# selkies-project/selkies

Measured on NVIDIA H100. Metric: 4K frames/sec encoded, higher is better.
Workload: dtype u8

## Files before the change

### selkies_b200/csrc/b2v_api.cu

```cuda
#include <condition_variable>
#include <cstdarg>
#include <cstdio>
#include <cstring>
#include <deque>
#include <mutex>
#include <thread>
#include <vector>

#include <sys/prctl.h>
#include <time.h>

#include "../../include/b2video.h"
#include "b2v_internal.h"
#include "h264_encoder.h"
#include "jpeg.h"

using namespace b2v;

static thread_local char g_err[512] = "";
static int fail(int code, const char* fmt, ...) {
  va_list ap; va_start(ap, fmt); vsnprintf(g_err, sizeof g_err, fmt, ap); va_end(ap);
  return code;
}
#define CK(call)                                                                              \
  do { cudaError_t e_ = (call);                                                               \
       if (e_ != cudaSuccess) return fail(B2V_ECUDA, "%s -> %s (%s:%d)", #call, cudaGetErrorString(e_), __FILE__, __LINE__); \
  } while (0)

namespace {

constexpr int kMaxSlots = 16;
constexpr int kOutHead = 64;
constexpr size_t kFirstChunk = 256 << 10;

struct Job {
  int out_idx; int in_slot; int frame_id; int is_key; int64_t capture_ns; int64_t pts; int hdr_w, hdr_h;
  bool timing;
};

inline int64_t now_ns() {
  timespec ts; clock_gettime(CLOCK_MONOTONIC, &ts);
  return (int64_t)ts.tv_sec * 1000000000LL + ts.tv_nsec;
}

constexpr int64_t kSpinNs = 30000, kSleepNs = 25000, kGiveUpNs = 30LL * 1000000000LL;
inline cudaError_t wait_event_polling(cudaEvent_t ev, bool* slept) {
  const int64_t t0 = now_ns();
  for (;;) {
    const cudaError_t e = cudaEventQuery(ev);
    if (e != cudaErrorNotReady) return e;
    const int64_t waited = now_ns() - t0;
    if (waited < kSpinNs) {
      for (int i = 0; i < 16; i++) __builtin_ia32_pause();
    } else if (waited > kGiveUpNs) {
      return cudaErrorLaunchTimeout;
    } else {
      *slept = true;
      timespec ts{0, (long)kSleepNs};
      nanosleep(&ts, nullptr);
    }
  }
}

enum : uint8_t { SLOT_FREE = 0, SLOT_ACQUIRED = 1, SLOT_IN_FLIGHT = 2 };

struct Session {
  b2v_settings cfg{};
  int device = 0;
  int src_w = 0, src_h = 0, dst_w = 0, dst_h = 0, coded_w = 0, coded_h = 0;
  bool encode = true, timing = false, timing_csc_only = false;
  cudaStream_t st_copy = nullptr, st_enc = nullptr, st_out = nullptr, st_pack = nullptr;

  int n_slots = 4;
  uint8_t* host_slot[kMaxSlots] = {};
  uint8_t* dev_slot[kMaxSlots] = {};
  cudaEvent_t ev_h2d[kMaxSlots] = {};
  uint8_t slot_state[kMaxSlots] = {};
  size_t frame_bytes = 0;
  std::vector<uint8_t*> resident;
  Tap *d_tx = nullptr, *d_ty = nullptr;
  uint8_t* d_cur = nullptr;
  Encoder* enc = nullptr;
  JpegEncoder* jenc = nullptr;
  bool jpeg = false;
  uint8_t* d_au[kMaxSlots] = {};
  uint8_t* h_out[kMaxSlots] = {};
  cudaEvent_t ev_enc[kMaxSlots] = {}, ev_out[kMaxSlots] = {};
  bool out_free[kMaxSlots] = {};
  AuLayout lay{};
  int out_next = 0;
  int ring_next = 0;
  cudaEvent_t ev_timer[2] = {};
  unsigned long long* d_csc_ts = nullptr;

  uint32_t frame_id = 0;
  int64_t frames_since_idr = 0;
  bool want_idr = true;
  double fps = 60.0;
  int bitrate_kbps = 8000;
  int qp_fixed = 26;

  cudaEvent_t ev_t[kMaxSlots][6] = {};

  b2v_cb cb = nullptr; void* user = nullptr;
  std::mutex mu;
  std::mutex submit_mu;
  std::condition_variable cv_slot, cv_job, cv_done;
  std::deque<Job> jobs;
  int64_t submitted = 0, delivered = 0;
  bool stopping = false;
  bool resizing = false;
  bool failed = false; char fail_msg[256] = "";
  std::thread out_thread;
  b2v_stats stats{};
};

int round16(int v) { return (v + 15) & ~15; }

bool size_ok(int w, int h) { return w >= 16 && h >= 16 && w <= 7680 && h <= 4320 && !(w & 1) && !(h & 1); }

int alloc_geometry(Session* s) {
  s->coded_w = s->encode ? round16(s->dst_w) : s->dst_w;
  s->coded_h = s->encode ? round16(s->dst_h) : s->dst_h;
  s->frame_bytes = (size_t)s->src_w * s->src_h * 4;
  for (int i = 0; i < s->n_slots; i++) {
    CK(cudaHostAlloc((void**)&s->host_slot[i], s->frame_bytes, cudaHostAllocDefault));
    CK(cudaMalloc((void**)&s->dev_slot[i], s->frame_bytes));
    s->slot_state[i] = SLOT_FREE;
  }
  CK(cudaMalloc((void**)&s->d_cur, (size_t)s->coded_w * s->coded_h * 3 / 2));
  if (s->dst_w != s->src_w || s->dst_h != s->src_h) {
    std::vector<Tap> tx(s->dst_w), ty(s->dst_h);
    make_taps_host(tx.data(), s->dst_w, s->src_w);
    make_taps_host(ty.data(), s->dst_h, s->src_h);
    CK(cudaMalloc((void**)&s->d_tx, sizeof(Tap) * s->dst_w));
    CK(cudaMalloc((void**)&s->d_ty, sizeof(Tap) * s->dst_h));
    CK(cudaMemcpy(s->d_tx, tx.data(), sizeof(Tap) * s->dst_w, cudaMemcpyHostToDevice));
    CK(cudaMemcpy(s->d_ty, ty.data(), sizeof(Tap) * s->dst_h, cudaMemcpyHostToDevice));
  }
  if (s->encode && s->jpeg) {
    JpegConfig jc{};
    jc.width = s->dst_w; jc.height = s->dst_h; jc.coded_w = s->coded_w; jc.coded_h = s->coded_h;
    jc.stripe_rows = s->cfg.stripe_rows > 0 ? s->cfg.stripe_rows : (s->coded_h / 16 + 7) / 8;
    jc.quality = s->cfg.crf > 0 ? s->cfg.crf : 60; jc.paint_quality = s->cfg.paintover_crf > 0 ? s->cfg.paintover_crf : 90;
    jc.paint_trigger = s->cfg.paintover_trigger_frames > 0 ? s->cfg.paintover_trigger_frames : 0;
    int rc = jpeg_create(&jc, &s->jenc);
    if (rc) return fail(rc, "jpeg_create failed: %s", jpeg_last_error());
    s->lay = jpeg_layout(s->jenc);
  } else if (s->encode) {
    EncoderConfig ec{};
    ec.width = s->dst_w; ec.height = s->dst_h; ec.coded_w = s->coded_w; ec.coded_h = s->coded_h;
    ec.slice_rows = s->cfg.slice_rows;
    ec.stripe_rows = s->cfg.stripe_rows > 0 ? s->cfg.stripe_rows : 0;
    ec.idr_slice_mbs = s->cfg.idr_slice_mbs;
    int rc = encoder_create(&ec, &s->enc);
    if (rc) return fail(rc, "encoder_create failed: %s", encoder_last_error());
    s->lay = encoder_layout(s->enc);
  }
  for (int i = 0; i < s->n_slots; i++) {
    if (s->encode) {
      CK(cudaMalloc((void**)&s->d_au[i], s->lay.cap));
      CK(cudaHostAlloc((void**)&s->h_out[i], s->lay.cap + kOutHead, cudaHostAllocDefault));
    }
    s->out_free[i] = true;
  }
  return 0;
}

void free_geometry(Session* s) {
  for (int i = 0; i < kMaxSlots; i++) {
    if (s->host_slot[i]) cudaFreeHost(s->host_slot[i]);
    if (s->dev_slot[i]) cudaFree(s->dev_slot[i]);
    if (s->d_au[i]) cudaFree(s->d_au[i]);
    if (s->h_out[i]) cudaFreeHost(s->h_out[i]);
    s->host_slot[i] = s->dev_slot[i] = s->d_au[i] = s->h_out[i] = nullptr;
  }
  for (auto p : s->resident) if (p) cudaFree(p);
  s->resident.clear();
  if (s->d_cur) cudaFree(s->d_cur);
  if (s->d_tx) cudaFree(s->d_tx);
  if (s->d_ty) cudaFree(s->d_ty);
  s->d_cur = nullptr; s->d_tx = nullptr; s->d_ty = nullptr;
  if (s->enc) { encoder_destroy(s->enc); s->enc = nullptr; }
  if (s->jenc) { jpeg_destroy(s->jenc); s->jenc = nullptr; }
}

CscParams csc_params(Session* s, const uint8_t* d_bgra, int stride, uint8_t* d_nv12) {
  CscParams p{};
  p.src = d_bgra; p.src_w = s->src_w; p.src_h = s->src_h; p.src_stride = stride;
  p.dst_w = s->dst_w; p.dst_h = s->dst_h; p.coded_w = s->coded_w; p.coded_h = s->coded_h;
  p.out_y = d_nv12; p.out_uv = d_nv12 + (size_t)s->coded_w * s->coded_h;
  p.tx = s->d_tx; p.ty = s->d_ty;
  p.matrix = s->jpeg ? 1 : 0;
  return p;
}

int wait_au(Session* s, const Job& j, int64_t* ns_event, bool* slept) {
  const int64_t tw = now_ns();
  const cudaError_t se = wait_event_polling(s->encode ? s->ev_out[j.out_idx] : s->ev_enc[j.out_idx], slept);
  *ns_event = now_ns() - tw;
  if (!s->encode) return 0;
  uint8_t* base = s->h_out[j.out_idx];
  const AuHeader* ah = (const AuHeader*)base;
  const int size = ah->size;
  const size_t doff = (size_t)s->lay.data_off;
  if (se != cudaSuccess || size < 0 || (size_t)size + doff > s->lay.cap || ah->overflow) {
    std::lock_guard<std::mutex> lk(s->mu);
    if (!s->failed) snprintf(s->fail_msg, sizeof s->fail_msg, "encode pipeline failed on frame %d: %s (size %d, overflow %d)", j.frame_id,
                             se != cudaSuccess ? cudaGetErrorString(se) : "invalid access unit", size, ah->overflow);
    s->failed = true;
    return 0;
  }
  if ((size_t)size + doff > kFirstChunk && size > 0) {
    size_t have = kFirstChunk;
    cudaMemcpyAsync(base + have, s->d_au[j.out_idx] + have, doff + (size_t)size - have, cudaMemcpyDeviceToHost, s->st_out);
    cudaStreamSynchronize(s->st_out);
    std::lock_guard<std::mutex> lk(s->mu);
    s->stats.d2h_bytes += (int64_t)(doff + size - have);
  }
  return size;
}

void add_timing(Session* s, const Job& j, bool have_au) {
  cudaEvent_t* ev = s->ev_t[j.out_idx];
  float ms[6] = {0, 0, 0, 0, 0, 0};
  cudaEventElapsedTime(&ms[0], ev[0], ev[1]);
  const bool stages = s->encode && !s->timing_csc_only;
  if (stages) {
    for (int k = 1; k < 5; k++) cudaEventElapsedTime(&ms[k], ev[k], ev[k + 1]);
    cudaEventElapsedTime(&ms[5], ev[0], ev[5]);
  } else ms[5] = ms[0];
  std::lock_guard<std::mutex> lk(s->mu);
  s->stats.ms_csc += ms[0]; s->stats.n_csc++;
  if (have_au) {
    const AuHeader* ah = (const AuHeader*)s->h_out[j.out_idx];
    if (ah->csc_t1 > ah->csc_t0 && ah->csc_t0 != 0) { s->stats.ms_csc_device += (double)(ah->csc_t1 - ah->csc_t0) * 1e-6; s->stats.n_csc_device++; }
  }
  if (stages) {
    if (j.is_key) { s->stats.ms_intra += ms[1]; s->stats.n_intra++; }
    else { s->stats.ms_inter += ms[1]; s->stats.n_inter++; }
    s->stats.ms_cavlc += ms[2]; s->stats.n_cavlc++;
    s->stats.ms_slice += ms[3]; s->stats.n_slice++;
    s->stats.ms_pack += ms[4]; s->stats.n_pack++;
  }
  s->stats.ms_total_gpu += ms[5];
}

void put_pixelflux_header(uint8_t* h, const Job& j, int y0, int bh) {
  h[0] = 0x04; h[1] = j.is_key ? 1 : 0;
  h[2] = (uint8_t)(j.frame_id >> 8); h[3] = (uint8_t)j.frame_id;
  h[4] = (uint8_t)(y0 >> 8); h[5] = (uint8_t)y0;
  h[6] = (uint8_t)(j.hdr_w >> 8); h[7] = (uint8_t)j.hdr_w;
  h[8] = (uint8_t)(bh >> 8); h[9] = (uint8_t)bh;
}

int64_t deliver(Session* s, const Job& j, int size, std::vector<BandEntry>& tab, int64_t* ns_cb) {
  uint8_t* base = s->h_out[j.out_idx];
  uint8_t* au = base + s->lay.data_off;
  const int qp = ((const AuHeader*)base)->qp;
  int rows = j.hdr_h;
  if (s->lay.n_bands == 0) {
    tab.assign(1, BandEntry{0, size, 1, 0});
  } else {
    tab.resize(s->lay.n_bands);
    memcpy(tab.data(), base + sizeof(AuHeader), sizeof(BandEntry) * s->lay.n_bands);
    rows = s->lay.band_rows * 16;
  }
  const bool hdr = s->cfg.header_mode == B2V_HDR_PIXELFLUX;
  int64_t bytes = 0;
  for (int b = 0; b < (int)tab.size(); b++) {
    const BandEntry& be = tab[b];
    if (!be.coded || be.size <= 0 || (long long)be.off + be.size > size) continue;
    const int y0 = b * rows, bh = (y0 + rows <= j.hdr_h) ? rows : j.hdr_h - y0;
    b2v_frame f{};
    f.data = au + be.off; f.size = be.size;
    if (hdr && s->jpeg) {
      uint8_t* h = au + be.off - 4;
      h[0] = (uint8_t)(j.frame_id >> 8); h[1] = (uint8_t)j.frame_id; h[2] = (uint8_t)(y0 >> 8); h[3] = (uint8_t)y0;
      f.data = h; f.size += 4;
    } else if (hdr) {
      put_pixelflux_header(au + be.off - 10, j, y0, bh);
      f.data = au + be.off - 10; f.size += 10;
    }
    f.frame_id = j.frame_id; f.is_key = j.is_key; f.qp = qp; f.pts90k = j.pts; f.capture_ns = j.capture_ns;
    f.y_start = y0; f.height = bh;
    bytes += f.size;
    if (s->cb) { const int64_t tc = now_ns(); s->cb(&f, s->user); *ns_cb += now_ns() - tc; }
  }
  return bytes;
}

void output_loop(Session* s) {
  cudaSetDevice(s->device);
  prctl(PR_SET_TIMERSLACK, 1000UL, 0, 0, 0);
  std::vector<BandEntry> tab;
  for (;;) {
    Job j;
    {
      std::unique_lock<std::mutex> lk(s->mu);
      if (s->jobs.empty() && !s->stopping) {
        const int64_t t0 = now_ns();
        s->cv_job.wait(lk, [&] { return s->stopping || !s->jobs.empty(); });
        s->stats.ns_wait_job += now_ns() - t0;
      }
      if (s->jobs.empty()) { if (s->stopping) return; continue; }
      j = s->jobs.front(); s->jobs.pop_front();
    }
    int64_t ns_event = 0, ns_cb = 0, bytes = 0; bool slept = false;
    const int size = wait_au(s, j, &ns_event, &slept);
    if (j.timing) add_timing(s, j, size > 0);
    if (size > 0) bytes = deliver(s, j, size, tab, &ns_cb);
    {
      std::lock_guard<std::mutex> lk(s->mu);
      if (j.in_slot >= 0) s->slot_state[j.in_slot] = SLOT_FREE;
      s->out_free[j.out_idx] = true;
      s->delivered++;
      s->stats.frames_delivered++;
      s->stats.bytes_out += bytes;
      if (j.is_key) s->stats.key_frames++;
      s->stats.ns_wait_event += ns_event; s->stats.ns_callback += ns_cb;
      if (ns_event > s->stats.ns_wait_event_max) s->stats.ns_wait_event_max = ns_event;
      if (slept) s->stats.n_event_sleeps++;
    }
    s->cv_slot.notify_all();
    s->cv_done.notify_all();
  }
}

int submit_failed(Session* s, int out_idx, int in_slot, cudaError_t e, const char* what) {
  {
    std::lock_guard<std::mutex> lk(s->mu);
    if (!s->failed) snprintf(s->fail_msg, sizeof s->fail_msg, "%s -> %s", what, cudaGetErrorString(e));
    s->failed = true;
    if (out_idx >= 0) { s->out_free[out_idx] = true; s->submitted--; s->stats.frames_submitted--; }
    if (in_slot >= 0) s->slot_state[in_slot] = SLOT_FREE;
  }
  s->cv_slot.notify_all(); s->cv_done.notify_all();
  return fail(B2V_ECUDA, "%s", s->fail_msg);
}
#define CKS(call)                                                                              \
  do { cudaError_t e_ = (call); if (e_ != cudaSuccess) return submit_failed(s, out_idx, in_slot, e_, #call); } while (0)

int submit_common(Session* s, const uint8_t* d_bgra, int stride, int in_slot, int64_t capture_ns) {
  int out_idx = 0;
  Job j{};
  EncodeFrameParams fp{};
  const int64_t t_enter = now_ns();
  int64_t t_slot = 0;
  {
    std::unique_lock<std::mutex> lk(s->mu);
    out_idx = s->out_next;
    s->cv_slot.wait(lk, [&] { return s->out_free[out_idx] || s->stopping || s->failed; });
    if (s->failed || s->stopping) {
      if (in_slot >= 0) s->slot_state[in_slot] = SLOT_FREE;
      lk.unlock(); s->cv_slot.notify_all();
      return s->failed ? fail(B2V_ECUDA, "%s", s->fail_msg) : fail(B2V_ESTATE, "session is stopping");
    }
    t_slot = now_ns() - t_enter;
    s->stats.ns_wait_out_slot += t_slot;
    s->out_free[out_idx] = false;
    s->out_next = (s->out_next + 1) % s->n_slots;
    bool idr = s->want_idr || (s->cfg.gop > 0 && s->frames_since_idr >= s->cfg.gop);
    s->want_idr = false;
    s->frames_since_idr = idr ? 1 : s->frames_since_idr + 1;
    j.out_idx = out_idx; j.in_slot = in_slot; j.frame_id = (int)(s->frame_id & 0xffff); j.is_key = idr;
    j.capture_ns = capture_ns;
    int ifps = (int)s->fps; if (ifps < 1) ifps = 1;
    j.pts = (int64_t)j.frame_id * (90000 / ifps);
    j.hdr_w = s->dst_w; j.hdr_h = s->dst_h;
    j.timing = s->timing && (!s->timing_csc_only || (s->frame_id & 3) == 0);
    s->frame_id++;
    fp.idr = idr;
    fp.rc_mode = s->cfg.rc_mode;
    fp.qp_fixed = s->qp_fixed;
    fp.paint_trigger = s->cfg.paintover_trigger_frames > 0 ? s->cfg.paintover_trigger_frames : 0;
    fp.paint_qp = s->cfg.paintover_crf;
    fp.paint_burst = s->cfg.paintover_burst_frames > 0 ? s->cfg.paintover_burst_frames : 1;
    fp.target_bits = (int64_t)((double)s->bitrate_kbps * 1000.0 / (s->fps > 0 ? s->fps : 60.0));
    s->submitted++;
    s->stats.frames_submitted++;
  }
  CscParams cp = csc_params(s, d_bgra, stride, s->d_cur);
  cudaEvent_t* ev = j.timing ? s->ev_t[out_idx] : nullptr;
  if (ev && s->d_csc_ts && s->encode) {
    cp.ts = s->d_csc_ts + 2 * out_idx;
    cudaMemsetAsync(cp.ts, 0xFF, sizeof(unsigned long long), s->st_enc);
    cudaMemsetAsync(cp.ts + 1, 0, sizeof(unsigned long long), s->st_enc);
  }
  if (ev) cudaEventRecord(ev[0], s->st_enc);
  int nl = launch_csc(cp, s->st_enc);
  if (ev) cudaEventRecord(ev[1], s->st_enc);
  cudaStream_t st_done = s->st_enc;
  if (s->encode && s->jpeg) {
    nl += jpeg_encode(s->jenc, s->d_cur, s->d_au[out_idx], j.is_key, s->st_enc);
  } else if (s->encode) {
    fp.cur = s->d_cur; fp.au = s->d_au[out_idx]; fp.ev = s->timing_csc_only ? nullptr : ev; fp.csc_ts = cp.ts;
    fp.st_pack = fp.ev ? nullptr : s->st_pack;
    nl += encoder_encode(s->enc, &fp, s->st_enc);
    if (fp.st_pack) st_done = fp.st_pack;
  }
  CKS(cudaEventRecord(s->ev_enc[out_idx], st_done));
  if (s->encode) {
    CKS(cudaStreamWaitEvent(s->st_out, s->ev_enc[out_idx], 0));
    const size_t first = s->lay.cap < kFirstChunk ? s->lay.cap : kFirstChunk;
    CKS(cudaMemcpyAsync(s->h_out[out_idx], s->d_au[out_idx], first, cudaMemcpyDeviceToHost, s->st_out));
    CKS(cudaEventRecord(s->ev_out[out_idx], s->st_out));
    std::lock_guard<std::mutex> lk(s->mu);
    s->stats.d2h_bytes += (int64_t)first;
  }
  CKS(cudaGetLastError());
  {
    std::lock_guard<std::mutex> lk(s->mu);
    s->stats.kernel_launches += nl;
    s->stats.ns_submit += now_ns() - t_enter - t_slot;
    s->jobs.push_back(j);
  }
  s->cv_job.notify_one();
  return 0;
}

void release_session(Session* s) {
  cudaSetDevice(s->device);
  cudaDeviceSynchronize();
  free_geometry(s);
  for (int i = 0; i < kMaxSlots; i++) {
    if (s->ev_h2d[i]) cudaEventDestroy(s->ev_h2d[i]);
    if (s->ev_enc[i]) cudaEventDestroy(s->ev_enc[i]);
    if (s->ev_out[i]) cudaEventDestroy(s->ev_out[i]);
    for (cudaEvent_t e : s->ev_t[i]) if (e) cudaEventDestroy(e);
  }
  if (s->ev_timer[0]) cudaEventDestroy(s->ev_timer[0]);
  if (s->ev_timer[1]) cudaEventDestroy(s->ev_timer[1]);
  if (s->d_csc_ts) cudaFree(s->d_csc_ts);
  if (s->st_copy) cudaStreamDestroy(s->st_copy);
  if (s->st_enc) cudaStreamDestroy(s->st_enc);
  if (s->st_out) cudaStreamDestroy(s->st_out);
  if (s->st_pack) cudaStreamDestroy(s->st_pack);
  delete s;
}

int bench_csc(Session* s, int32_t n_resident, int32_t iters, float* ms_per_launch, bool burst) {
  if (!s || n_resident <= 0 || n_resident > (int)s->resident.size() || iters <= 0 || !ms_per_launch) return fail(B2V_EINVAL, "bad argument");
  int rc = b2v_flush(s);
  if (rc) return rc;
  std::lock_guard<std::mutex> sub(s->submit_mu);
  CK(cudaSetDevice(s->device));
  std::vector<uint8_t*> outs(n_resident, nullptr);
  size_t ob = (size_t)s->coded_w * s->coded_h * 3 / 2;
  for (auto& o : outs) CK(cudaMalloc((void**)&o, ob));
  for (int i = 0; i < n_resident; i++) launch_csc(csc_params(s, s->resident[i], s->src_w * 4, outs[i]), s->st_enc);
  CK(cudaStreamSynchronize(s->st_enc));
  const int pairs = burst ? 1 : iters;
  std::vector<cudaEvent_t> e0(pairs), e1(pairs);
  for (int i = 0; i < pairs; i++) { cudaEventCreate(&e0[i]); cudaEventCreate(&e1[i]); }
  if (burst) cudaEventRecord(e0[0], s->st_enc);
  for (int i = 0; i < iters; i++) {
    int k = i % n_resident;
    if (!burst) cudaEventRecord(e0[i], s->st_enc);
    launch_csc(csc_params(s, s->resident[k], s->src_w * 4, outs[k]), s->st_enc);
    if (!burst) cudaEventRecord(e1[i], s->st_enc);
  }
  if (burst) cudaEventRecord(e1[0], s->st_enc);
  CK(cudaStreamSynchronize(s->st_enc));
  double total = 0;
  for (int i = 0; i < pairs; i++) { float ms = 0; cudaEventElapsedTime(&ms, e0[i], e1[i]); total += ms; cudaEventDestroy(e0[i]); cudaEventDestroy(e1[i]); }
  for (auto o : outs) cudaFree(o);
  CK(cudaGetLastError());
  *ms_per_launch = (float)(total / iters);
  return 0;
}

}

extern "C" {

int b2v_abi_version(void) { return B2V_ABI_VERSION; }
const char* b2v_last_error(void) { return g_err; }

int b2v_device_count(void) {
  int n = 0;
  if (cudaGetDeviceCount(&n) != cudaSuccess) return 0;
  return n;
}

int b2v_create(const b2v_settings* cfg, b2v_cb cb, void* user, void** out) {
  if (!cfg || !out) return fail(B2V_EINVAL, "null argument");
  int sw = cfg->src_w, sh = cfg->src_h;
  int dw = cfg->dst_w > 0 ? cfg->dst_w : sw, dh = cfg->dst_h > 0 ? cfg->dst_h : sh;
  if (!size_ok(sw, sh)) return fail(B2V_EINVAL, "source size %dx%d unsupported (even, 16..7680 x 16..4320)", sw, sh);
  if (!size_ok(dw, dh)) return fail(B2V_EINVAL, "encoded size %dx%d unsupported", dw, dh);
  if (cfg->idr_slice_mbs < 0) return fail(B2V_EINVAL, "idr_slice_mbs %d out of range (0 = default, n > 0 macroblocks per slice)", cfg->idr_slice_mbs);
  int ndev = 0;
  CK(cudaGetDeviceCount(&ndev));
  if (cfg->device < 0 || cfg->device >= ndev) return fail(B2V_EINVAL, "device %d out of range (%d devices)", cfg->device, ndev);
  CK(cudaSetDevice(cfg->device));
  Session* s = new Session();
  s->cfg = *cfg; s->device = cfg->device;
  s->src_w = sw; s->src_h = sh; s->dst_w = dw; s->dst_h = dh;
  s->encode = !(cfg->flags & B2V_FLAG_NO_ENCODE);
  s->jpeg = (cfg->flags & B2V_FLAG_JPEG) != 0;
  s->timing = (cfg->flags & (B2V_FLAG_TIMING | B2V_FLAG_TIMING_CSC)) != 0;
  s->timing_csc_only = s->timing && !(cfg->flags & B2V_FLAG_TIMING);
  s->n_slots = cfg->ring_slots > 0 ? cfg->ring_slots : 4;
  if (s->n_slots < 2) s->n_slots = 2;
  if (s->n_slots > kMaxSlots) s->n_slots = kMaxSlots;
  s->fps = cfg->fps > 0 ? cfg->fps : 60.0;
  s->bitrate_kbps = cfg->bitrate_kbps > 0 ? cfg->bitrate_kbps : 8000;
  s->qp_fixed = cfg->crf >= 0 ? cfg->crf : 26;
  if (s->qp_fixed > 51) s->qp_fixed = 51;
  s->cb = cb; s->user = user;
  cudaStreamCreateWithFlags(&s->st_copy, cudaStreamNonBlocking);
  cudaStreamCreateWithFlags(&s->st_enc, cudaStreamNonBlocking);
  cudaStreamCreateWithFlags(&s->st_out, cudaStreamNonBlocking);
  cudaStreamCreateWithFlags(&s->st_pack, cudaStreamNonBlocking);
  for (int i = 0; i < kMaxSlots; i++) {
    cudaEventCreateWithFlags(&s->ev_h2d[i], cudaEventDisableTiming);
    cudaEventCreateWithFlags(&s->ev_enc[i], cudaEventDisableTiming);
    cudaEventCreateWithFlags(&s->ev_out[i], cudaEventDisableTiming);
  }
  for (auto& evs : s->ev_t) for (cudaEvent_t& e : evs) cudaEventCreate(&e);
  cudaEventCreate(&s->ev_timer[0]); cudaEventCreate(&s->ev_timer[1]);
  if (s->timing && (cfg->flags & B2V_FLAG_DEVICE_TIMER)) cudaMalloc((void**)&s->d_csc_ts, sizeof(unsigned long long) * 2 * kMaxSlots);
  int rc = alloc_geometry(s);
  if (rc) { release_session(s); return rc; }
  s->out_thread = std::thread(output_loop, s);
  *out = s;
  return 0;
}

void b2v_destroy(void* h) {
  if (!h) return;
  Session* s = (Session*)h;
  b2v_flush(h);
  {
    std::lock_guard<std::mutex> lk(s->mu);
    s->stopping = true;
  }
  s->cv_job.notify_all(); s->cv_slot.notify_all();
  if (s->out_thread.joinable()) s->out_thread.join();
  release_session(s);
}

void* b2v_ring_acquire(void* h, int32_t* slot) {
  Session* s = (Session*)h;
  if (!s || !slot) { fail(B2V_EINVAL, "null argument"); return nullptr; }
  std::unique_lock<std::mutex> lk(s->mu);
  if ((s->resizing || s->slot_state[s->ring_next] != SLOT_FREE) && !s->stopping && !s->failed) {
    const int64_t t0 = now_ns();
    s->cv_slot.wait(lk, [&] { return s->stopping || s->failed || (!s->resizing && s->slot_state[s->ring_next] == SLOT_FREE); });
    s->stats.ns_wait_ring += now_ns() - t0;
  }
  if (s->failed) { fail(B2V_ECUDA, "%s", s->fail_msg); return nullptr; }
  if (s->stopping) { fail(B2V_ESTATE, "session is stopping"); return nullptr; }
  const int found = s->ring_next;
  s->ring_next = (found + 1) % s->n_slots;
  s->slot_state[found] = SLOT_ACQUIRED;
  *slot = found;
  return s->host_slot[found];
}

int b2v_ring_release(void* h, int32_t slot) {
  Session* s = (Session*)h;
  if (!s || slot < 0 || slot >= s->n_slots) return fail(B2V_EINVAL, "bad slot");
  {
    std::lock_guard<std::mutex> lk(s->mu);
    if (s->slot_state[slot] != SLOT_ACQUIRED || (slot + 1) % s->n_slots != s->ring_next) return fail(B2V_ESTATE, "slot %d is not the most recently acquired one", slot);
    s->slot_state[slot] = SLOT_FREE;
    s->ring_next = slot;
  }
  s->cv_slot.notify_all();
  return 0;
}

int b2v_ring_submit(void* h, int32_t slot, int32_t stride, int64_t capture_ns) {
  Session* s = (Session*)h;
  if (!s || slot < 0 || slot >= s->n_slots) return fail(B2V_EINVAL, "bad slot");
  if (stride <= 0) stride = s->src_w * 4;
  if (stride < s->src_w * 4 || (size_t)stride * s->src_h > s->frame_bytes) return fail(B2V_EINVAL, "stride %d does not fit the slot", stride);
  std::lock_guard<std::mutex> sub(s->submit_mu);
  {
    std::lock_guard<std::mutex> lk(s->mu);
    if (s->slot_state[slot] != SLOT_ACQUIRED) return fail(B2V_ESTATE, "slot %d was not acquired (double submit?)", slot);
    s->slot_state[slot] = SLOT_IN_FLIGHT;
  }
  const int64_t t0 = now_ns();
  const int out_idx = -1, in_slot = slot;
  CKS(cudaSetDevice(s->device));
  CKS(cudaMemcpyAsync(s->dev_slot[slot], s->host_slot[slot], (size_t)stride * s->src_h, cudaMemcpyHostToDevice, s->st_copy));
  CKS(cudaEventRecord(s->ev_h2d[slot], s->st_copy));
  CKS(cudaStreamWaitEvent(s->st_enc, s->ev_h2d[slot], 0));
  {
    std::lock_guard<std::mutex> lk(s->mu);
    s->stats.h2d_bytes += (int64_t)stride * s->src_h;
    s->stats.ns_submit += now_ns() - t0;
  }
  return submit_common(s, s->dev_slot[slot], stride, slot, capture_ns);
}

int b2v_resident_upload(void* h, int32_t index, const void* bgra, int32_t stride) {
  Session* s = (Session*)h;
  if (!s || index < 0 || index >= 1024 || !bgra) return fail(B2V_EINVAL, "bad argument");
  if (stride <= 0) stride = s->src_w * 4;
  std::lock_guard<std::mutex> sub(s->submit_mu);
  CK(cudaSetDevice(s->device));
  if ((int)s->resident.size() <= index) s->resident.resize(index + 1, nullptr);
  if (!s->resident[index]) CK(cudaMalloc((void**)&s->resident[index], s->frame_bytes));
  CK(cudaMemcpy2D(s->resident[index], (size_t)s->src_w * 4, bgra, stride, (size_t)s->src_w * 4, s->src_h, cudaMemcpyHostToDevice));
  return 0;
}

int b2v_submit_resident(void* h, int32_t index, int64_t capture_ns) {
  Session* s = (Session*)h;
  if (!s || index < 0 || index >= (int)s->resident.size() || !s->resident[index]) return fail(B2V_EINVAL, "resident frame %d not uploaded", index);
  std::lock_guard<std::mutex> sub(s->submit_mu);
  CK(cudaSetDevice(s->device));
  return submit_common(s, s->resident[index], s->src_w * 4, -1, capture_ns);
}

int b2v_flush(void* h) {
  Session* s = (Session*)h;
  if (!s) return fail(B2V_EINVAL, "null handle");
  std::unique_lock<std::mutex> lk(s->mu);
  s->cv_done.wait(lk, [&] { return s->delivered >= s->submitted; });
  if (s->failed) return fail(B2V_ECUDA, "%s", s->fail_msg);
  return 0;
}

int b2v_set_framerate(void* h, double fps) {
  Session* s = (Session*)h;
  if (!s || !(fps > 0) || fps > 1000) return fail(B2V_EINVAL, "fps out of range");
  std::lock_guard<std::mutex> lk(s->mu);
  s->fps = fps;
  return 0;
}
int b2v_set_bitrate_kbps(void* h, int32_t kbps) {
  Session* s = (Session*)h;
  if (!s || kbps <= 0) return fail(B2V_EINVAL, "bitrate out of range");
  std::lock_guard<std::mutex> lk(s->mu);
  s->bitrate_kbps = kbps;
  return 0;
}
int b2v_set_qp(void* h, int32_t qp) {
  Session* s = (Session*)h;
  if (!s || qp < 0 || qp > 51) return fail(B2V_EINVAL, "qp out of range");
  std::lock_guard<std::mutex> lk(s->mu);
  s->qp_fixed = qp;
  return 0;
}
int b2v_set_gop(void* h, int32_t frames) {
  Session* s = (Session*)h;
  if (!s) return fail(B2V_EINVAL, "null handle");
  std::lock_guard<std::mutex> lk(s->mu);
  s->cfg.gop = frames;
  return 0;
}
int b2v_request_idr(void* h) {
  Session* s = (Session*)h;
  if (!s) return fail(B2V_EINVAL, "null handle");
  std::lock_guard<std::mutex> lk(s->mu);
  s->want_idr = true;
  return 0;
}

int b2v_set_resolution(void* h, int32_t sw, int32_t sh, int32_t dw, int32_t dh) {
  Session* s = (Session*)h;
  if (!s) return fail(B2V_EINVAL, "null handle");
  if (dw <= 0) dw = sw;
  if (dh <= 0) dh = sh;
  if (!size_ok(sw, sh) || !size_ok(dw, dh)) return fail(B2V_EINVAL, "size unsupported");
  std::lock_guard<std::mutex> sub(s->submit_mu);
  {
    std::unique_lock<std::mutex> lk(s->mu);
    s->cv_done.wait(lk, [&] { return s->delivered >= s->submitted; });
    if (s->failed) return fail(B2V_ECUDA, "%s", s->fail_msg);
    for (int i = 0; i < s->n_slots; i++)
      if (s->slot_state[i] == SLOT_ACQUIRED) return fail(B2V_ESTATE, "ring slot %d is still held by the producer: submit or release it before resizing", i);
    s->resizing = true;
  }
  CK(cudaSetDevice(s->device));
  CK(cudaDeviceSynchronize());
  free_geometry(s);
  s->src_w = sw; s->src_h = sh; s->dst_w = dw; s->dst_h = dh;
  const int rc = alloc_geometry(s);
  std::lock_guard<std::mutex> lk(s->mu);
  if (rc) {
    s->failed = true;
    snprintf(s->fail_msg, sizeof s->fail_msg, "b2v_set_resolution(%dx%d -> %dx%d): %.150s", sw, sh, dw, dh, g_err);
  }
  s->want_idr = true;
  s->out_next = 0; s->ring_next = 0;
  s->resizing = false;
  s->cv_slot.notify_all();
  return rc;
}

int b2v_get_stats(void* h, b2v_stats* out) {
  Session* s = (Session*)h;
  if (!s || !out) return fail(B2V_EINVAL, "null argument");
  std::lock_guard<std::mutex> lk(s->mu);
  *out = s->stats;
  return 0;
}
int b2v_reset_stats(void* h) {
  Session* s = (Session*)h;
  if (!s) return fail(B2V_EINVAL, "null handle");
  std::lock_guard<std::mutex> lk(s->mu);
  memset(&s->stats, 0, sizeof s->stats);
  return 0;
}
int b2v_coded_size(void* h, int32_t* cw, int32_t* ch) {
  Session* s = (Session*)h;
  if (!s) return fail(B2V_EINVAL, "null handle");
  if (cw) *cw = s->coded_w;
  if (ch) *ch = s->coded_h;
  return 0;
}

int b2v_csc_nv12(void* h, const void* bgra, int32_t stride, void* nv12) {
  Session* s = (Session*)h;
  if (!s || !bgra || !nv12) return fail(B2V_EINVAL, "null argument");
  if (stride <= 0) stride = s->src_w * 4;
  int rc = b2v_flush(h);
  if (rc) return rc;
  std::lock_guard<std::mutex> sub(s->submit_mu);
  CK(cudaSetDevice(s->device));
  uint8_t *d_in = nullptr, *d_out = nullptr;
  size_t out_bytes = (size_t)s->dst_w * s->dst_h * 3 / 2;
  CK(cudaMalloc((void**)&d_in, (size_t)s->src_w * 4 * s->src_h));
  CK(cudaMalloc((void**)&d_out, out_bytes));
  CK(cudaMemcpy2DAsync(d_in, (size_t)s->src_w * 4, bgra, stride, (size_t)s->src_w * 4, s->src_h, cudaMemcpyHostToDevice, s->st_enc));
  CscParams p = csc_params(s, d_in, s->src_w * 4, d_out);
  p.coded_w = s->dst_w; p.coded_h = s->dst_h;
  p.out_uv = d_out + (size_t)s->dst_w * s->dst_h;
  launch_csc(p, s->st_enc);
  CK(cudaMemcpyAsync(nv12, d_out, out_bytes, cudaMemcpyDeviceToHost, s->st_enc));
  CK(cudaStreamSynchronize(s->st_enc));
  cudaFree(d_in); cudaFree(d_out);
  CK(cudaGetLastError());
  return 0;
}

int b2v_get_recon(void* h, void* nv12) {
  Session* s = (Session*)h;
  if (!s || !nv12) return fail(B2V_EINVAL, "null argument");
  if (!s->encode || !s->enc) return fail(B2V_ESTATE, "no H.264 reconstruction in this session (B2V_FLAG_NO_ENCODE / B2V_FLAG_JPEG)");
  int rc = b2v_flush(h);
  if (rc) return rc;
  std::lock_guard<std::mutex> sub(s->submit_mu);
  CK(cudaSetDevice(s->device));
  CK(cudaStreamSynchronize(s->st_enc));
  CK(cudaMemcpy(nv12, encoder_recon(s->enc), (size_t)s->coded_w * s->coded_h * 3 / 2, cudaMemcpyDeviceToHost));
  return 0;
}

int b2v_bench_csc(void* h, int32_t n_resident, int32_t iters, float* ms_per_launch) {
  return bench_csc((Session*)h, n_resident, iters, ms_per_launch, false);
}

int b2v_timer_start(void* h) {
  Session* s = (Session*)h;
  if (!s) return fail(B2V_EINVAL, "null handle");
  int rc = b2v_flush(h);
  if (rc) return rc;
  std::lock_guard<std::mutex> sub(s->submit_mu);
  CK(cudaSetDevice(s->device));
  CK(cudaDeviceSynchronize());
  CK(cudaEventRecord(s->ev_timer[0], s->st_enc));
  return 0;
}

int b2v_timer_stop(void* h, float* ms) {
  Session* s = (Session*)h;
  if (!s || !ms) return fail(B2V_EINVAL, "null argument");
  int rc = b2v_flush(h);
  if (rc) return rc;
  std::lock_guard<std::mutex> sub(s->submit_mu);
  CK(cudaSetDevice(s->device));
  CK(cudaEventRecord(s->ev_timer[1], s->st_enc));
  CK(cudaEventSynchronize(s->ev_timer[1]));
  CK(cudaEventElapsedTime(ms, s->ev_timer[0], s->ev_timer[1]));
  return 0;
}

int b2v_bench_csc_burst(void* h, int32_t n_resident, int32_t iters, float* ms_per_launch) {
  return bench_csc((Session*)h, n_resident, iters, ms_per_launch, true);
}

}
```

Baseline: 6895.

## Run color conversion on a separate stream with double-buffered NV12 frames

Moves the BGRA-to-NV12 conversion onto its own stream and double-buffers the converted frame, so conversion of frame N+1 can overlap encoding of frame N. Events gate encoder start on conversion completion and buffer reuse on encoder completion. This applies only to the H.264 path without timing. It costs one extra NV12 buffer plus cross-stream event overhead, and it changes how the pack stream is chosen for the non-timing path.

```diff
diff --git a/selkies_b200/csrc/b2v_api.cu b/selkies_b200/csrc/b2v_api.cu
--- a/selkies_b200/csrc/b2v_api.cu
+++ b/selkies_b200/csrc/b2v_api.cu
@@ -69,7 +69,7 @@
   int device = 0;
   int src_w = 0, src_h = 0, dst_w = 0, dst_h = 0, coded_w = 0, coded_h = 0;
   bool encode = true, timing = false, timing_csc_only = false;
-  cudaStream_t st_copy = nullptr, st_enc = nullptr, st_out = nullptr, st_pack = nullptr;
+  cudaStream_t st_copy = nullptr, st_enc = nullptr, st_out = nullptr, st_pack = nullptr, st_csc = nullptr;
 
   int n_slots = 4;
   uint8_t* host_slot[kMaxSlots] = {};
@@ -79,7 +79,8 @@
   size_t frame_bytes = 0;
   std::vector<uint8_t*> resident;
   Tap *d_tx = nullptr, *d_ty = nullptr;
-  uint8_t* d_cur = nullptr;
+  uint8_t* d_cur[2] = {};
+  cudaEvent_t ev_csc[2] = {}, ev_cur_free[2] = {};
   Encoder* enc = nullptr;
   JpegEncoder* jenc = nullptr;
   bool jpeg = false;
@@ -119,6 +120,8 @@
 
 bool size_ok(int w, int h) { return w >= 16 && h >= 16 && w <= 7680 && h <= 4320 && !(w & 1) && !(h & 1); }
 
+bool two_stream(const Session* s) { return s->encode && !s->jpeg && !(s->cfg.flags & B2V_FLAG_TIMING); }
+
 int alloc_geometry(Session* s) {
   s->coded_w = s->encode ? round16(s->dst_w) : s->dst_w;
   s->coded_h = s->encode ? round16(s->dst_h) : s->dst_h;
@@ -128,7 +131,7 @@
     CK(cudaMalloc((void**)&s->dev_slot[i], s->frame_bytes));
     s->slot_state[i] = SLOT_FREE;
   }
-  CK(cudaMalloc((void**)&s->d_cur, (size_t)s->coded_w * s->coded_h * 3 / 2));
+  for (int b = 0; b < (two_stream(s) ? 2 : 1); b++) CK(cudaMalloc((void**)&s->d_cur[b], (size_t)s->coded_w * s->coded_h * 3 / 2));
   if (s->dst_w != s->src_w || s->dst_h != s->src_h) {
     std::vector<Tap> tx(s->dst_w), ty(s->dst_h);
     make_taps_host(tx.data(), s->dst_w, s->src_w);
@@ -177,10 +180,10 @@
   }
   for (auto p : s->resident) if (p) cudaFree(p);
   s->resident.clear();
-  if (s->d_cur) cudaFree(s->d_cur);
+  for (uint8_t*& c : s->d_cur) { if (c) cudaFree(c); c = nullptr; }
   if (s->d_tx) cudaFree(s->d_tx);
   if (s->d_ty) cudaFree(s->d_ty);
-  s->d_cur = nullptr; s->d_tx = nullptr; s->d_ty = nullptr;
+  s->d_tx = nullptr; s->d_ty = nullptr;
   if (s->enc) { encoder_destroy(s->enc); s->enc = nullptr; }
   if (s->jenc) { jpeg_destroy(s->jenc); s->jenc = nullptr; }
 }
@@ -342,7 +345,7 @@
   do { cudaError_t e_ = (call); if (e_ != cudaSuccess) return submit_failed(s, out_idx, in_slot, e_, #call); } while (0)
 
 int submit_common(Session* s, const uint8_t* d_bgra, int stride, int in_slot, int64_t capture_ns) {
-  int out_idx = 0;
+  int out_idx = 0, par = 0;
   Job j{};
   EncodeFrameParams fp{};
   const int64_t t_enter = now_ns();
@@ -369,6 +372,7 @@
     j.pts = (int64_t)j.frame_id * (90000 / ifps);
     j.hdr_w = s->dst_w; j.hdr_h = s->dst_h;
     j.timing = s->timing && (!s->timing_csc_only || (s->frame_id & 3) == 0);
+    par = (int)(s->frame_id & 1);
     s->frame_id++;
     fp.idr = idr;
     fp.rc_mode = s->cfg.rc_mode;
@@ -380,24 +384,35 @@
     s->submitted++;
     s->stats.frames_submitted++;
   }
-  CscParams cp = csc_params(s, d_bgra, stride, s->d_cur);
+  const bool ahead = two_stream(s);
+  const int cb = ahead ? par : 0;
+  cudaStream_t st_csc = ahead ? s->st_csc : s->st_enc;
+  if (ahead) CKS(cudaStreamWaitEvent(st_csc, s->ev_cur_free[cb], 0));
+  CscParams cp = csc_params(s, d_bgra, stride, s->d_cur[cb]);
   cudaEvent_t* ev = j.timing ? s->ev_t[out_idx] : nullptr;
   if (ev && s->d_csc_ts && s->encode) {
     cp.ts = s->d_csc_ts + 2 * out_idx;
-    cudaMemsetAsync(cp.ts, 0xFF, sizeof(unsigned long long), s->st_enc);
-    cudaMemsetAsync(cp.ts + 1, 0, sizeof(unsigned long long), s->st_enc);
-  }
-  if (ev) cudaEventRecord(ev[0], s->st_enc);
-  int nl = launch_csc(cp, s->st_enc);
-  if (ev) cudaEventRecord(ev[1], s->st_enc);
+    cudaMemsetAsync(cp.ts, 0xFF, sizeof(unsigned long long), st_csc);
+    cudaMemsetAsync(cp.ts + 1, 0, sizeof(unsigned long long), st_csc);
+  }
+  if (ev) cudaEventRecord(ev[0], st_csc);
+  int nl = launch_csc(cp, st_csc);
+  if (ev) cudaEventRecord(ev[1], st_csc);
+  if (ahead) {
+    CKS(cudaEventRecord(s->ev_csc[cb], st_csc));
+    CKS(cudaStreamWaitEvent(s->st_enc, s->ev_csc[cb], 0));
+  }
   cudaStream_t st_done = s->st_enc;
   if (s->encode && s->jpeg) {
-    nl += jpeg_encode(s->jenc, s->d_cur, s->d_au[out_idx], j.is_key, s->st_enc);
+    nl += jpeg_encode(s->jenc, s->d_cur[cb], s->d_au[out_idx], j.is_key, s->st_enc);
   } else if (s->encode) {
-    fp.cur = s->d_cur; fp.au = s->d_au[out_idx]; fp.ev = s->timing_csc_only ? nullptr : ev; fp.csc_ts = cp.ts;
-    fp.st_pack = fp.ev ? nullptr : s->st_pack;
+    fp.cur = s->d_cur[cb]; fp.au = s->d_au[out_idx]; fp.ev = ahead ? nullptr : ev; fp.csc_ts = cp.ts;
+    fp.st_pack = ahead ? s->st_pack : nullptr;
     nl += encoder_encode(s->enc, &fp, s->st_enc);
-    if (fp.st_pack) st_done = fp.st_pack;
+    if (ahead) {
+      st_done = s->st_pack;
+      CKS(cudaEventRecord(s->ev_cur_free[cb], s->st_enc));
+    }
   }
   CKS(cudaEventRecord(s->ev_enc[out_idx], st_done));
   if (s->encode) {
@@ -429,6 +444,10 @@
     if (s->ev_out[i]) cudaEventDestroy(s->ev_out[i]);
     for (cudaEvent_t e : s->ev_t[i]) if (e) cudaEventDestroy(e);
   }
+  for (int b = 0; b < 2; b++) {
+    if (s->ev_csc[b]) cudaEventDestroy(s->ev_csc[b]);
+    if (s->ev_cur_free[b]) cudaEventDestroy(s->ev_cur_free[b]);
+  }
   if (s->ev_timer[0]) cudaEventDestroy(s->ev_timer[0]);
   if (s->ev_timer[1]) cudaEventDestroy(s->ev_timer[1]);
   if (s->d_csc_ts) cudaFree(s->d_csc_ts);
@@ -436,6 +455,7 @@
   if (s->st_enc) cudaStreamDestroy(s->st_enc);
   if (s->st_out) cudaStreamDestroy(s->st_out);
   if (s->st_pack) cudaStreamDestroy(s->st_pack);
+  if (s->st_csc) cudaStreamDestroy(s->st_csc);
   delete s;
 }
 
@@ -513,6 +533,11 @@
   cudaStreamCreateWithFlags(&s->st_enc, cudaStreamNonBlocking);
   cudaStreamCreateWithFlags(&s->st_out, cudaStreamNonBlocking);
   cudaStreamCreateWithFlags(&s->st_pack, cudaStreamNonBlocking);
+  cudaStreamCreateWithFlags(&s->st_csc, cudaStreamNonBlocking);
+  for (int b = 0; b < 2; b++) {
+    cudaEventCreateWithFlags(&s->ev_csc[b], cudaEventDisableTiming);
+    cudaEventCreateWithFlags(&s->ev_cur_free[b], cudaEventDisableTiming);
+  }
   for (int i = 0; i < kMaxSlots; i++) {
     cudaEventCreateWithFlags(&s->ev_h2d[i], cudaEventDisableTiming);
     cudaEventCreateWithFlags(&s->ev_enc[i], cudaEventDisableTiming);
@@ -588,7 +613,7 @@
   CKS(cudaSetDevice(s->device));
   CKS(cudaMemcpyAsync(s->dev_slot[slot], s->host_slot[slot], (size_t)stride * s->src_h, cudaMemcpyHostToDevice, s->st_copy));
   CKS(cudaEventRecord(s->ev_h2d[slot], s->st_copy));
-  CKS(cudaStreamWaitEvent(s->st_enc, s->ev_h2d[slot], 0));
+  CKS(cudaStreamWaitEvent(two_stream(s) ? s->st_csc : s->st_enc, s->ev_h2d[slot], 0));
   {
     std::lock_guard<std::mutex> lk(s->mu);
     s->stats.h2d_bytes += (int64_t)stride * s->src_h;
@@ -766,6 +791,7 @@
   CK(cudaSetDevice(s->device));
   CK(cudaDeviceSynchronize());
   CK(cudaEventRecord(s->ev_timer[0], s->st_enc));
+  CK(cudaStreamWaitEvent(s->st_csc, s->ev_timer[0], 0));
   return 0;
 }
 
```

After: 6858, median of 6. No clear change (-0.5%).
